# NethermindEth/latticefold

Hardware: AMD Instinct MI355X
Metric: folding-prover steps/sec (one NIFSProver::prove per step), GoldilocksRingNTT (higher is better)
Workload: dtype u64; 1 GPU; C4: GoldilocksRingNTT R1CS->CCS, m=N=2^20 rows, wit_len=262144, L=4, B=2^16, b=2, K=16, kappa=26, t=3; parallelism=replicas x1

## Files before the change

### latticefold_amd/api.py

```python
import ctypes as C
import os

import numpy as np

RE = 24
P = 2**64 - 2**32 + 1
RING_IDS = {"goldilocks": 0, "babybear": 1}
RING_WORDS = {"goldilocks": 24, "babybear": 72}
RING_TAU = {"goldilocks": 3, "babybear": 9}
FORMS = {"ntt": 0, "coeff": 1}
_HERE = os.path.dirname(os.path.abspath(__file__))
_SO = os.path.join(_HERE, "liblfhip.so")

u64p = C.POINTER(C.c_uint64)
u32p = C.POINTER(C.c_uint32)


EXCHANGE_FN = C.CFUNCTYPE(C.c_int, C.c_void_p, u64p, u64p, C.c_size_t)


class LfError(RuntimeError):
    def __init__(self, code, where=""):
        self.code = code
        msg = _lib().lf_strerror(code).decode() if _LIB is not None else str(code)
# ... 515 lines not shown
    def phase_ms(self):
        out = (C.c_float * 8)()
        _chk(_lib().lf_last_phase_ms(self.h, out), "lf_last_phase_ms")
        return {_lib().lf_phase_name(i).decode(): float(out[i]) for i in range(8)}

    def fold_paths(self):
        m = C.c_uint()
        _chk(_lib().lf_last_fold_paths(self.h, C.byref(m)), "lf_last_fold_paths")
        return m.value

    def lin_split_rounds(self):
        m = C.c_uint()
        _chk(_lib().lf_last_lin_split_rounds(self.h, C.byref(m)), "lf_last_lin_split_rounds")
        return m.value

    def fold_split_rounds(self):
        m = C.c_uint()
        _chk(_lib().lf_last_fold_split_rounds(self.h, C.byref(m)), "lf_last_fold_split_rounds")
        return m.value

    def timeline(self):
        names, ms = C.create_string_buffer(32 * 64), (C.c_double * 64)()
        n = _lib().lf_last_timeline(self.h, names, ms, 64)
        if n < 0:
            raise LfError(n, "lf_last_timeline")
        return [(names.raw[32 * i:32 * i + 32].split(b"\0")[0].decode(), float(ms[i])) for i in range(n)]

    def device_memory(self):
        f, t = C.c_size_t(), C.c_size_t()
        _chk(_lib().lf_device_memory(self.h, C.byref(f), C.byref(t)), "lf_device_memory")
# ... 574 lines not shown
```

### latticefold_amd/csrc/lf_capi.cpp

```cpp
#include "lf_ring_host.h"
#include <thread>
#include <vector>

const char *lf_strerror(int code) {
    switch (code) {
        case LF_OK: return "ok";
        case LF_ERR_INVALID: return "invalid argument / wrong length";
        case LF_ERR_HIP: return "HIP runtime error (no GPU or out of device memory)";
        case LF_ERR_UNSUPPORTED: return "unsupported parameter";
        case LF_ERR_BAD_TABLES: return "ring tables are not a ring isomorphism";
        case LF_ERR_NORM: return "witness coefficient exceeds the decomposition bound";
        case LF_ERR_SIZE_BOUNDS: return "invalid size bounds (m must be >= wit_len*L, power of two)";
        case LF_ERR_STATE: return "call sequence misuse";
        case LF_ERR_REJECT: return "verifier rejected the proof";
    }
    return "unknown error";
}
const char *lf_phase_name(int i) { return (i >= 0 && i < LF_N_PHASES) ? PHASE_NAMES[i] : ""; }

static int install_tables(lf_ctx *c, u64 nonres, const u64 *y) {
    CrtTables T;
    if (build_crt_tables(nonres, y, T) != 0) return LF_ERR_BAD_TABLES;
    c->ring.T = T;
    c->dcrt = make_dev_crt(T);
// ... 1009 lines not shown
        if (n >= max_marks) break;
        const char *w = m.first;
        while (*w == ' ') w++;
        snprintf(names + 32 * n, 32, "%s", w);
        ms[n++] = m.second;
    }
    return n;
}
int lf_abi_version(void) { return LFHIP_ABI_VERSION; }
int lf_debug_i8_prof(uint64_t *out64) {
    if (!out64) return LF_ERR_INVALID;
    return getenv("LF_I8G_PROF") ? ajtai_i8g_read_prof((unsigned long long *)out64) : ajtai_i8_read_prof((unsigned long long *)out64);
}
extern "C" int lfdbg_i8g_wg(unsigned int *out512) { return out512 ? ajtai_i8g_read_wg(out512) : -1; }
extern "C" unsigned lfdbg_i8g_planes_base(int ring, uint64_t base) { return ajtai_i8g_planes_base(ring == LF_RING_BABYBEAR ? ajtai_i8_babybear() : ajtai_i8_goldilocks(), base); }
int lf_last_fold_paths(lf_ctx *c, unsigned *sv_round_mask) {
    if (!c || !sv_round_mask) return LF_ERR_INVALID;
    *sv_round_mask = c->core_any().sv_round_mask;
    return LF_OK;
}
int lf_last_fold_split_rounds(lf_ctx *c, unsigned *round_mask) {
    if (!c || !round_mask) return LF_ERR_INVALID;
    *round_mask = c->core_any().fold_split_mask;
    return LF_OK;
}
int lf_last_lin_split_rounds(lf_ctx *c, unsigned *rounds) {
    if (!c || !rounds) return LF_ERR_INVALID;
    *rounds = c->bb ? 0u : c->lin_split_rounds;
    return LF_OK;
}
// ... 45 lines not shown
```

### latticefold_amd/csrc/lf_common.h

```cpp
#pragma once
#include <hip/hip_runtime.h>

#include <stdlib.h>

#include <atomic>

#include "../../include/lfhip.h"

#define HIPCHK(x)                                    \
    do {                                             \
        hipError_t e__ = (x);                        \
        if (e__ != hipSuccess) return LF_ERR_HIP;    \
    } while (0)
#define RET(x)                      \
    do {                            \
        int rc__ = (x);             \
        if (rc__ != LF_OK) return rc__; \
    } while (0)

extern "C" void lfplus_scratch_trim(int device);
template <class T> static inline hipError_t lf_dev_malloc(T **p, size_t bytes) {
    hipError_t e = hipMalloc((void **)p, bytes);
    if (e != hipErrorOutOfMemory) return e;
    (void)hipGetLastError();
// ... 43 lines not shown
    uint64_t *w_ccs = nullptr;
    size_t w_bytes = 0;
};

int lf_planes_alloc(lf_ctx *ctx, size_t bytes, int32_t **out);
void lf_planes_release(lf_ctx *ctx, size_t bytes, int32_t *p);
int lf_ctx_device(const lf_ctx *ctx);


struct Tunables {
    bool lin_u_eval = false, fold_unfused = false, fold_no_lut = false, fold_tab_r1 = false, theta_eval = false, fold_no_r4tab = false, fold_no_r5tab = false;
    bool fold_rounds_no_split = false;
    bool fold_sv_no_split = false;
    bool lin_no_split = false;
    size_t lin_split_min = (size_t)1 << 17;
    size_t fold_split_min = 8192;
    bool force_exchange = false;
    bool device_transcript = false;
    bool shard_plain_rounds = false;
    int shard_two_lanes = -1;
    size_t shard_lin_min = 16384;
    size_t shard_fold_min = 2048;
    long i8_wgs = 0;
    bool lin_no_r1cs = false;
    bool lin_no_small = false;
    size_t dot_min = 4096;
    bool dot_valu = false;
    bool fold_no_sv = false;
    size_t sv_min = 65536;
    int sv_rounds = 3;
// ... 1 lines not shown
    size_t fuse_min = 16384, lut_min = (size_t)1 << 17, tab_min = 16384;
    size_t r5_min = 8192;
    size_t tail_n = 2048;
    static Tunables read(size_t lut_min_default) {
        Tunables t;
        t.lut_min = lut_min_default;
        const char *e;
        t.lin_u_eval = getenv("LF_LIN_U_EVAL") != nullptr;
        t.fold_unfused = getenv("LF_FOLD_UNFUSED") != nullptr;
        t.fold_no_lut = getenv("LF_FOLD_NO_LUT") != nullptr;
        t.fold_tab_r1 = getenv("LF_FOLD_TAB_R1") != nullptr;
        t.fold_no_r4tab = getenv("LF_FOLD_NO_R4TAB") != nullptr;
        t.fold_no_r5tab = getenv("LF_FOLD_NO_R5TAB") != nullptr;
        t.lin_no_split = getenv("LF_LIN_NO_SPLIT") != nullptr;
        t.fold_sv_no_split = getenv("LF_FOLD_SV_NO_SPLIT") != nullptr;
        t.fold_rounds_no_split = getenv("LF_FOLD_ROUNDS_NO_SPLIT") != nullptr;
        if (const char *e = getenv("LF_LIN_SPLIT_MIN")) t.lin_split_min = (size_t)atoll(e);
        if (const char *e = getenv("LF_FOLD_SPLIT_MIN")) t.fold_split_min = (size_t)atoll(e);
        t.theta_eval = getenv("LF_THETA_EVAL") != nullptr;
        t.no_tail = getenv("LF_NO_TAIL") != nullptr;
        t.fold_no_sv = getenv("LF_FOLD_NO_SV") != nullptr;
        t.dot_valu = getenv("LF_DOT_VALU") != nullptr;
        if ((e = getenv("LF_DOT_MIN"))) t.dot_min = (size_t)atoll(e);
        t.lin_no_small = getenv("LF_LIN_NO_SMALL") != nullptr;
        t.lin_no_r1cs = getenv("LF_LIN_NO_R1CS") != nullptr;
        if ((e = getenv("LF_FOLD_SV_MIN"))) t.sv_min = (size_t)atoll(e);
        if ((e = getenv("LF_FOLD_SV_ROUNDS"))) t.sv_rounds = atoi(e);
        if ((e = getenv("LF_I8_WGS"))) t.i8_wgs = atol(e);
        if ((e = getenv("LF_SHARD_TWO_LANES"))) t.shard_two_lanes = atoi(e) != 0;
        if ((e = getenv("LF_SHARD_LIN_MIN"))) t.shard_lin_min = (size_t)atoll(e);
// ... 79 lines not shown
```

### latticefold_amd/csrc/lf_ctx.h

```cpp
#pragma once
#include <hip/hip_runtime.h>
#include <assert.h>
#include <string.h>

#include <atomic>
#include <chrono>
#include <condition_variable>
#include <functional>
#include <future>
#include <thread>
#include <map>
#include <memory>
#include <mutex>
#include <set>
#include <string>
#include <vector>

#include "../../include/lfhip.h"
#include "bb_capi.h"
#include "lf_ctx_core.h"
#include "lf_common.h"
#include "lf_dist.h"
#include "lf_kernels.h"
#include "lf_sb.h"
#include "lf_verify.h"

using namespace lf;

namespace lf {
void launch_fix_many(const DevCrt &t, const u64 *in, size_t ld_in, u64 *out, size_t ld_out, size_t n_in, u32 rows3, Fq3Const r, hipStream_t s);
}

#include <stdio.h>
#include <stdlib.h>
static bool lf_trace_on() { static int v = -1; if (v < 0) v = getenv("LF_TRACE") ? 1 : 0; return v == 1; }
#define LF_TRACE(c, msg)                                                              \
    do {                                                                              \
        if (lf_trace_on()) {                                                          \
// ... 103 lines not shown
    std::atomic<int> io_jobs{0};
    inline CtxCoreBase &core_any();
    bool have_ccs_any() { return core_any().have_ccs; }
    const lf_params &params_any() { return core_any().P; }
    size_t n_any() { return core_any().n; }
    size_t m_any() { return core_any().m; }
    size_t N_any() { return core_any().N; }
    HostRing ring;
    DevCrt dcrt;
    LaneWorker lane1;
    int agreed_two_lanes = -1;
    bool two_lanes_ok = false;
    lfdist::Comm comm[2];
    lfdist::Comm &cm() { assert(t_lane < 2); return comm[t_lane]; }
    bool ccs_general = false;
    size_t shc_r0 = (size_t)-1, shc_rcnt = 0, shc_lo = 0, shc_hi = 0;
    LinCombDesc desc{};
    std::vector<std::pair<const char *, double>> tl_marks;
    const lf_witness *bits_wit[2] = {nullptr, nullptr};
    u32 *bits_ptr[2] = {nullptr, nullptr};
    hipEvent_t bits_ev[2] = {nullptr, nullptr};
    hipEvent_t ev_yR = nullptr, ev_yL = nullptr;
    u64 *h_pin2 = nullptr;
    size_t h_pin2_words = 0;
    int pin2(size_t words) {
        if (words <= h_pin2_words) return LF_OK;
        if (h_pin2) (void)hipHostFree(h_pin2);
        h_pin2 = nullptr; h_pin2_words = 0;
        if (hipHostMalloc((void **)&h_pin2, words * 8) != hipSuccess) return LF_ERR_HIP;
        h_pin2_words = words;
        return LF_OK;
    }
    hipStream_t st_aux = nullptr;
    hipEvent_t ev_aux = nullptr;
    u64 *h_aux = nullptr;
    unsigned lin_split_rounds = 0;

    unsigned char *stage[LF_NLANES] = {nullptr, nullptr, nullptr};
    size_t stage_off[LF_NLANES] = {0, 0, 0};
    static constexpr size_t STAGE_BYTES = (size_t)1 << 20;
    int h2d_small(void *dst, const void *src, size_t bytes) {
        unsigned char *&ring = stage[t_lane];
        if (!ring && hipHostMalloc((void **)&ring, STAGE_BYTES, hipHostMallocDefault) != hipSuccess) { ring = nullptr; return LF_ERR_HIP; }
        const size_t need = (bytes + 63) & ~(size_t)63;
        if (need > STAGE_BYTES) {
            HIPCHK(hipMemcpyAsync(dst, src, bytes, hipMemcpyHostToDevice, stream()));
            HIPCHK(hipStreamSynchronize(stream()));
            return LF_OK;
        }
        if (stage_off[t_lane] + need > STAGE_BYTES) {
            HIPCHK(hipStreamSynchronize(stream()));
// ... 164 lines not shown
```

### latticefold_amd/csrc/lf_fold.cpp

```cpp
#include "lf_ring_host.h"

static int tail_host_rounds(lf_ctx *c, Transcript &tr, u32 epoch, u32 nr, u32 npts, bool dev_transcript, u64 *msgs, Fq3 *pt,
                            const std::function<void(u32)> *after_round = nullptr, u32 round0 = 0) {
    TailMail *mail = c->tail_mail;
    const auto t_start = std::chrono::steady_clock::now();
    double host_us = 0, wait_us = 0;
    auto t_mark = t_start;
    const bool tl_on = t_tl && t_tl->on;
    for (u32 i = 0; i < nr; i++) {
        u32 spins = 0;
        while (__atomic_load_n(&mail->msg_seq[i], __ATOMIC_ACQUIRE) != epoch) {
            __builtin_ia32_pause();
            if ((++spins & 0xfff) == 0) {
                if (__atomic_load_n(&mail->err, __ATOMIC_RELAXED) == epoch ||
                    std::chrono::duration<double>(std::chrono::steady_clock::now() - t_start).count() > 10.0) {
                    __atomic_store_n(&mail->abort_seq, epoch, __ATOMIC_RELEASE);
                    (void)hipStreamSynchronize(c->stream());
                    return LF_ERR_HIP;
                }
            }
        }
        if (tl_on) { auto nw = std::chrono::steady_clock::now(); wait_us += std::chrono::duration<double, std::micro>(nw - t_mark).count(); t_mark = nw; }
        u64 *evs = msgs + (size_t)i * npts * 24;
        memcpy(evs, (const void *)mail->msg[i], (size_t)npts * 24 * 8);
// ... 240 lines not shown
    od = od_host = c->round_out();
    if (!od) return LF_ERR_HIP;
    if (c->sh_world > 1) {
        RET(c->tbuf("fold_round_out", 5 * 24 + 8, &od_shard));
        od = od_shard;
    }
    const bool shard_tabs = shard_keep(c, 1, m);
    const size_t g_r0 = shard_tabs ? (size_t)c->sh_rank * (m / (size_t)c->sh_world) : 0, g_rcnt = shard_tabs ? m / (size_t)c->sh_world : (size_t)-1;
    size_t zc_lo = 0, zc_hi = n;
    if (shard_tabs) RET(shard_col_range(c, g_r0, g_rcnt, &zc_lo, &zc_hi));
    {
        hipStream_t s0 = c->stream(), s1 = (t_lane == 0) ? c->st_lane[1] : s0;
        u64 *zz1 = zz;
        if (s1 != s0) RET(c->tbuf("fold_zz1", (size_t)P.t * 24 * n, &zz1));
        RET(c->fork(s0, s1));
        for (int sd = 0; sd < 2; sd++) {
            hipStream_t st = sd ? s1 : s0;
            RET(side_mz(sd, st, sd ? zz1 : zz, sd ? "spmv_zaos_R" : "spmv_zaos_L", zc_lo, zc_hi, g_r0, g_rcnt));
            launch_add_fhat_comb(c->dcrt, S[sd].planes, N, K, d_ap + (size_t)sd * K * 3, G[sd], m, st, g_r0, g_rcnt);
        }
        RET(c->join(s1, s0));
    }
    { HostTimer ht(c); lfs::draw_mu_beta<GoldV>(tr, K2, P.s, mu, beta); }
    TL_MARK(" fold challenges");
    RET(powers_mu());
    RET(build_eq_dev(c, beta.data(), P.s, eqb));
    sv_split = !c->tn.fold_sv_no_split && P.s >= 4 && m >= 256;
    if (sv_split) {
        RET(c->tbuf("fold_svE1", 3 * (m / 2), &svE[0]));
        RET(c->tbuf("fold_svE2", 3 * (m / 4), &svE[1]));
        RET(c->tbuf("fold_svE3", 3 * (m / 8), &svE[2]));
        RET(build_eq_dev(c, beta.data() + 1, P.s - 1, svE[0]));
// ... 429 lines not shown
```

### latticefold_amd/csrc/lf_kernels.h

```cpp
#pragma once
#include "lf_ajtai_i8.h"
#include "lf_sv_rounds.h"
#include <hip/hip_runtime.h>

#include "lf_host.h"

namespace lf {

struct DevCrt {
    u64 nu;
    int nu2p40;
    u64 w4, w2, w10, w1, w7, w5, w11;
    int slot_of_pos[8], pos1[8], pos2[8];
    u64 tw1[8], tw2[8];
};
DevCrt make_dev_crt(const CrtTables &T);

struct Fq3Const { u64 c[3]; };

struct XbMat3 { u64 m[9]; };
void launch_aos_to_soa(const u64 *aos, u64 *soa, size_t n, hipStream_t s, u32 *flag = nullptr, const XbMat3 *Ti = nullptr);
void launch_soa_to_aos(const u64 *soa, u64 *aos, size_t n, hipStream_t s, const u32 *unless_flag = nullptr, const XbMat3 *T = nullptr);
void launch_ext_to_aos(const u64 *soa, u64 *aos, size_t n, hipStream_t s, const XbMat3 *T = nullptr);
void launch_slot_const_check(const u64 *tab, size_t n, u32 *flag, hipStream_t s);
// ... 33 lines not shown
                      u64 *zaos, u64 *out, size_t m, int accumulate, hipStream_t s, size_t r0 = 0, size_t rcnt = (size_t)-1);
void launch_spmv_t_eq(const DevCrt &t, const u32 *colptr, const u32 *rowidx, const u64 *val, const u64 *eq, size_t m,
                      u64 *q, size_t n, hipStream_t s, size_t c0 = 0, size_t ccnt = (size_t)-1 );
void launch_dot_batch(const DevCrt &t, const u64 *X, size_t ldx, u32 na, const u64 *Y, size_t ldy, u32 nb, size_t n,
                      u64 *partial, u64 *out, hipStream_t s);
size_t dot_partial_words(u32 na, u32 nb);
void launch_dot_eq(const DevCrt &t, const u64 *X, size_t ldx, u32 na, const u64 *eq, size_t ldeq, size_t n, u64 *partial,
                   u64 *out, hipStream_t s);
void launch_coef_eval(const DevCrt &t, const int32_t *planes, size_t n, const u64 *eq, size_t ldeq, u32 K, int mode_bits,
                      u64 *partial, u64 *out, hipStream_t s, size_t ldp = 0);
size_t coef_eval_partial_words(u32 K);
void launch_lincomb_z(const DevCrt &t, const u64 *z, size_t ldz, u32 K, const Fq3Const *coef_dev , u32 tt, size_t n,
                      u64 *out, hipStream_t s, u32 per_slot = 0);
void launch_add_fhat_comb(const DevCrt &t, const int32_t *planes, size_t n_planes, u32 K, const Fq3Const *apow_dev ,
                          u64 *G, size_t m, hipStream_t s, size_t r0 = 0, size_t rcnt = (size_t)-1 );

void launch_fix_ring(const DevCrt &t, const u64 *in, u64 *out, size_t n_in, Fq3Const r, hipStream_t s);
void launch_fix_fq3(const DevCrt &t, const u64 *in, u64 *out, size_t n_in, Fq3Const r, hipStream_t s);
size_t dot_i8_yb_bytes(size_t n);
size_t dot_i8_part_words(size_t n);
size_t dot_i8_tot_words();
int launch_dot_batch_i8(const DevCrt &t, const u64 *X, size_t ldx, u32 na, const u64 *Y, size_t ldy, u32 nb, size_t n, unsigned char *YB, int32_t *part,
                        long long *tot, u64 *out, hipStream_t s, bool y_packed = false, u32 nb_out = 0, u32 b0 = 0);
int launch_dot_pack_y(const u64 *X, const u64 *Y, size_t ldy, u32 nb, size_t n, unsigned char *YB, hipStream_t s);
void launch_vs_combine(const u64 *vs , u32 K, u64 *v , hipStream_t s);
void launch_fix_final(const DevCrt &t, const u64 *in , u32 rows3, Fq3Const r, u64 *out , hipStream_t s);

struct LinCombDesc {
    u32 t, q;
    u32 S_off[9];
// ... 114 lines not shown
```

### latticefold_amd/csrc/lf_kernels.hip

```cpp
#include "lf_kernels.h"

#include <stdlib.h>

#include "lf_kernels_dev.cuh"
#include "lf_sb.h"

namespace lf {


DevCrt make_dev_crt(const CrtTables &T) {
    DevCrt d;
    d.nu = T.nu; d.nu2p40 = T.nu_is_2p40;
    d.w4 = T.w4; d.w2 = T.w2; d.w10 = T.w10; d.w1 = T.w1; d.w7 = T.w7; d.w5 = T.w5; d.w11 = T.w11;
    for (int p = 0; p < 8; p++) {
        d.slot_of_pos[p] = T.slot_of_pos[p]; d.pos1[p] = T.pos1[p]; d.pos2[p] = T.pos2[p];
        d.tw1[p] = T.tw1[p]; d.tw2[p] = T.tw2[p];
    }
    return d;
}


__global__ void __launch_bounds__(256) k_modsum(const u64 *parts, u32 nparts, size_t words, u64 *out) {
    size_t w = (size_t)blockIdx.x * 256 + threadIdx.x;
    if (w >= words) return;
// ... 680 lines not shown
            const u64 *e = T[(d * NQ + q) * 16 + ((mg >> (4 * q)) & 15)];
            part = fq3_add(part, fq3_make(e[0], e[1], e[2]));
        }
        acc = v < 0 ? fq3_sub(acc, part) : fq3_add(acc, part);
    }
    st3(G, m, slot, row, acc);
}
void launch_add_fhat_comb(const DevCrt &t, const int32_t *planes, size_t n_planes, u32 K, const Fq3Const *apow_dev, u64 *G, size_t m,
                          hipStream_t s, size_t r0, size_t rcnt) {
    size_t r1 = rcnt == (size_t)-1 ? n_planes : (r0 + rcnt < n_planes ? r0 + rcnt : n_planes);
    if (rcnt == (size_t)-1) r0 = 0;
    if (r1 <= r0) return;
    if (K <= 16) hipLaunchKernelGGL(k_add_fhat_comb<4>, dim3(cdiv(r1 - r0, 256), 8), dim3(256), 0, s, planes, n_planes, K, apow_dev, G, m, r0, r1);
    else hipLaunchKernelGGL(k_add_fhat_comb<8>, dim3(cdiv(r1 - r0, 256), 8), dim3(256), 0, s, planes, n_planes, K, apow_dev, G, m, r0, r1);
}

template <bool NU>
__global__ void __launch_bounds__(256) k_fix(DevCrt t, const u64 *in, size_t ld_in, u64 *out, size_t ld_out, size_t n_out, Fq3Const r) {
    size_t j = (size_t)blockIdx.x * 256 + threadIdx.x;
    size_t row = blockIdx.y;
    if (j >= n_out) return;
    const u64 *p = in + row * 3 * ld_in;
    Fq3 rr = fq3_make(r.c[0], r.c[1], r.c[2]);
    ulonglong2 a0 = *(const ulonglong2 *)(p + 2 * j), a1 = *(const ulonglong2 *)(p + ld_in + 2 * j), a2 = *(const ulonglong2 *)(p + 2 * ld_in + 2 * j);
    Fq3 v0 = fq3_make(a0.x, a1.x, a2.x), v1 = fq3_make(a0.y, a1.y, a2.y);
    Fq3 res = fq3_add(v0, M3<NU>(fq3_sub(v1, v0), rr, t.nu));
    u64 *q = out + row * 3 * ld_out;
    q[j] = res.c[0]; q[ld_out + j] = res.c[1]; q[2 * ld_out + j] = res.c[2];
}
void launch_fix_ring(const DevCrt &t, const u64 *in, u64 *out, size_t n_in, Fq3Const r, hipStream_t s) {
// ... 67 lines not shown
```

### latticefold_amd/csrc/lf_prove.cpp

```cpp
#include "lf_ring_host.h"


static int run_lin_sumcheck(lf_ctx *c, Transcript &tr, const u64 *mz, const u64 *eqb, u64 *msgs , Fq3 *point, u64 *u_dev = nullptr,
                            const std::function<void(u32)> *after_round = nullptr, const Fq3 *beta = nullptr) {
    const lf_params &P = c->P;
    u32 deg = P.d + 1;
    size_t m = c->m;
    u64 *fx[2], *fe[2], *partial, *od;
    RET(c->tbuf("lin_fix0", (size_t)P.t * 24 * (m / 2), &fx[0]));
    RET(c->tbuf("lin_fix1", (size_t)P.t * 24 * (m / 4 ? m / 4 : 1), &fx[1]));
    RET(c->tbuf("lin_efix0", 3 * (m / 2), &fe[0]));
    RET(c->tbuf("lin_efix1", 3 * (m / 4 ? m / 4 : 1), &fe[1]));
    RET(c->tbuf("round_partial", round_partial_words(), &partial));
    od = c->round_out();
    if (!od) return LF_ERR_HIP;
    { HostTimer ht(c); lfs::sumcheck_prologue<GoldV>(tr, P.s, deg); }
    const u64 *cur = mz, *cure = eqb;
    size_t n = m;
    int flip = 0;
    const size_t Gw = (size_t)c->sh_world, gr = (size_t)c->sh_rank;
    bool sharded = shard_keep(c, 0, m);
    u64 *od_dev = nullptr;
    if (Gw > 1) RET(c->tbuf("lin_round_out", (size_t)(deg + 1) * 24 + 8, &od_dev));
    const u32 dT = P.d;
    const bool wide = P.t > 4 || P.d > 3;
    bool split = beta && Gw == 1 && !c->tn.lin_no_split && P.s >= 2 && m >= c->tn.lin_split_min && m >= 16 && dT >= 1 && deg <= 8;
    const GoldV hv{c->ring};
    lfs::SplitCoef<GoldV> sp = lfs::split_coef(hv, fq3_one(), beta ? beta[0] : fq3_one());
    if (split) RET(build_eq_dev(c, beta + 1, P.s - 1, fe[0]));
    c->lin_split_rounds = 0;
    for (u32 round = 1; round <= P.s; round++) {
        if (split && round >= 2) {
            const bool tail_next = !wide && !c->tn.no_tail && n <= c->tn.tail_n && n >= 4 && P.s - round + 1 <= TAIL_MAX_ROUNDS;
            const lfs::SplitCoef<GoldV> sp_next = lfs::split_coef(hv, c->ring.mul3(sp.c, lfs::eq1(hv, beta[round - 2], point[round - 2])), beta[round - 1]);
            if (tail_next || n < 8 || n / 2 < c->tn.lin_split_min || !sp_next.ok) {
                u64 *ex;
                RET(c->tbuf("lin_eexp", 3 * n, &ex));
                const Fq3 bi = beta[round - 2];
                launch_eq_expand(c->dcrt, cure, n / 2, n / 2, f3c(c->ring.mul3(sp.c, fq3_sub(fq3_one(), bi))), f3c(c->ring.mul3(sp.c, bi)), ex, n, c->stream());
                cure = ex;
                split = false;
            } else sp = sp_next;
        }
        if (!wide && !sharded && !c->tn.no_tail && round >= 2 && n <= c->tn.tail_n && n >= 4 && P.s - round + 1 <= TAIL_MAX_ROUNDS) {
            int trc = lin_tail_rounds(c, tr, cur, cure, n, fx[flip], partial, round, point, msgs, deg, after_round);
            if (trc == LF_OK) { cur = fx[flip]; n = 2; break; }
            if (trc != LF_ERR_UNSUPPORTED) return trc;
        }
        bool fused_now = false;
        const u64 *prev = cur, *preve = cure;
        size_t prevn = n;
        if (round > 1) {
            Fq3Const r = f3c(point[round - 2]);
            if (sharded) {
                const size_t e0 = gr * (n / Gw), ecnt = n / Gw;
                launch_fix_many(c->dcrt, cur + e0, n, fx[flip] + e0 / 2, n / 2, ecnt, P.t * 8, r, c->stream());
                launch_fix_many(c->dcrt, cure + e0, n, fe[flip] + e0 / 2, n / 2, ecnt, 1, r, c->stream());
            } else if (split || (Gw == 1 && n >= 8)) {
                fused_now = true;
            } else {
                launch_fix_many(c->dcrt, cur, n, fx[flip], n / 2, n, P.t * 8, r, c->stream());
                launch_fix_many(c->dcrt, cure, n, fe[flip], n / 2, n, 1, r, c->stream());
            }
            cur = fx[flip]; cure = split ? fe[(round - 1) & 1] : fe[flip];
            flip ^= 1;
            n /= 2;
            if (sharded && !shard_keep(c, 0, n)) {
                const size_t lcl = n / Gw;
                const GatherPart gp[2] = {{cur + gr * lcl, n, (u64 *)cur, (size_t)P.t * 24}, {cure + gr * lcl, n, (u64 *)cure, 3}};
                RET(gather_parts(c, gp, 2, lcl));
                sharded = false;
            }
        }
        u64 *ev = msgs + (size_t)(round - 1) * (deg + 1) * 24;
        if (sharded) {
            const size_t p0 = gr * (n / 2 / Gw), pcnt = n / 2 / Gw;
            launch_lin_round(c->dcrt, c->desc, cur + 2 * p0, n, cure + 2 * p0, n, 2 * pcnt, deg, partial, od_dev, c->stream(), c->lin_blocks);
            RET(exchange_modsum_dev(c, od_dev, (size_t)(deg + 1) * 24));
            HIPCHK(hipMemcpyAsync(od, od_dev, (size_t)(deg + 1) * 24 * 8, hipMemcpyDeviceToHost, c->stream()));
        } else if (split) {
            const u32 xmask = round == 1 ? (1u << (dT + 1)) - 1 : (((1u << (dT + 1)) - 1) & ~2u);
            if (round == 1) launch_lin_round(c->dcrt, c->desc, cur, n, fe[0], n / 2, n, deg, partial, od, c->stream(), c->lin_blocks, xmask);
            else launch_lin_round_fused(c->dcrt, c->desc, prev, prevn, preve, prevn / 2, f3c(point[round - 2]), (u64 *)cur, n, (u64 *)cure, n / 2, n, deg, partial, od, c->stream(),
                                        c->lin_blocks, xmask);
            if (round == 1) cure = fe[0];
        } else if (fused_now)
            launch_lin_round_fused(c->dcrt, c->desc, prev, prevn, preve, prevn, f3c(point[round - 2]), (u64 *)cur, n, (u64 *)cure, n, n, deg, partial, od, c->stream(), c->lin_blocks);
        else launch_lin_round(c->dcrt, c->desc, cur, n, cure, n, n, deg, partial, od, c->stream(), c->lin_blocks);
        RET(c->lane_sync());
        if (split) {
            HostTimer ht2(c);
            c->lin_split_rounds++;
            lfs::complete_lin_split(hv, sp, dT, od, round >= 2 ? msgs + (size_t)(round - 2) * (deg + 1) * 24 : nullptr, point[round >= 2 ? round - 2 : 0], ev);
        } else
        memcpy(ev, od, (size_t)(deg + 1) * 24 * 8);
        HostTimer ht(c);
        point[round - 1] = lfs::sumcheck_round<GoldV>(tr, ev, deg + 1);
        if (after_round) (*after_round)(round);
        if (round <= 2 || round == 4 || round == 8) TL_MARK_ROUND("  lin round", round);
    }
    TL_MARK("  lin rounds done");
    if (u_dev) launch_fix_final(c->dcrt, cur, P.t * 8, f3c(point[P.s - 1]), u_dev, c->stream());
    return LF_OK;
// ... 51 lines not shown
    RET(c->tbuf("lin_z", 24 * n, &z));
    RET(c->tbuf("lin_mz", (size_t)P.t * 24 * m, &mz));
    RET(c->tbuf("lin_eqb", 3 * m, &eqb));
    RET(c->tbuf("eq_r_R", 3 * m, &eqr));
    RET(c->tbuf("red_partial", 256 * 4096, &partial));
    RET(c->tbuf("lin_small", 4096, &od));
    RET(build_z(c, wit->planes, 1, 0, head.data(), z));
    TL_MARK("  lin z enqueued");
    std::vector<Fq3> beta(P.s);
    {
        HostTimer ht(c);
        tr.absorb_label("beta_s");
        for (u32 i = 0; i < P.s; i++) beta[i] = tr.get_challenge();
    }
    RET(build_eq_dev(c, beta.data(), P.s, eqb));
    {
        const size_t Gw = (size_t)c->sh_world;
        const bool rows_sliced = shard_keep(c, 0, m) && !c->tn.lin_u_eval;
        const size_t r0 = rows_sliced ? (size_t)c->sh_rank * (m / Gw) : 0, rcnt = rows_sliced ? m / Gw : m;
        if (c->ccs_general) {
            u64 *zaos;
            RET(c->tbuf("spmv_zaos", (size_t)P.t * n * 24, &zaos));
            launch_soa_to_aos(z, zaos, n, c->stream());
            for (u32 j = 0; j < P.t; j++)
                launch_spmv_rows(c->dcrt, 1, &c->d_rowptr[j], &c->d_col[j], &c->d_val[j], nullptr, 0, n, zaos, mz + (size_t)j * 24 * m, m, 0, c->stream(), r0, rcnt);
        } else
        for (u32 j = 0; j < P.t; j++)
            launch_spmv(c->dcrt, c->d_rowptr[j], c->d_col[j], c->d_val[j], z, n, mz + (size_t)j * 24 * m, m, 0, c->stream(), r0, rcnt);
    }
    std::vector<Fq3> pt(P.s);
    const bool u_eval = c->tn.lin_u_eval;
    TL_MARK("  lin Mz enqueued");
    struct VsSplit {
        bool armed = false, launched = false, failed = false;
// ... 24 lines not shown
    }
    const std::function<void(u32)> vs_hook = [&](u32 round) {
        if (!vsp.armed || round != vsp.J) return;
        Fq3Const *h = (Fq3Const *)c->h_aux;
        for (u32 i = 0; i < vsp.J; i++) h[i] = f3c(pt[i]);
        bool ok = hipMemcpyAsync(vsp.rd, h, vsp.J * sizeof(Fq3Const), hipMemcpyHostToDevice, c->st_aux) == hipSuccess;
        if (ok) {
            launch_build_eq2(c->dcrt, vsp.rd, vsp.J, vsp.scr, vsp.eqlo, c->st_aux);
            ok = hipStreamWaitEvent(c->st_aux, c->bits_ev[vsp.sd], 0) == hipSuccess &&
                 launch_sv_vs_blocks(c->bits_ptr[vsp.sd], c->N, vsp.eqlo, (size_t)1 << vsp.J, vsp.J, P.K, vsp.EB, vsp.part, c->st_aux) == 0 &&
                 hipEventRecord(c->ev_aux, c->st_aux) == hipSuccess;
        }
        vsp.launched = ok;
        vsp.failed = !ok;
    };
    RET(run_lin_sumcheck(c, tr, mz, eqb, proof, pt.data(), u_eval ? nullptr : od + 72, vsp.armed ? &vs_hook : nullptr, beta.data()));
    if (vsp.failed) { (void)hipStreamSynchronize(c->st_aux); return LF_ERR_HIP; }
    if (!vsp.launched) RET(build_eq_dev(c, pt.data(), P.s, eqr));
    u64 *v = proof + (size_t)P.s * (P.d + 2) * 24, *u = v + 3 * 24;
    {
        size_t i0, cnt;
        shard_slice(c, c->N, &i0, &cnt);
        c->vs_wit = nullptr;
        if (P.b == 2 && c->sh_world == 1 && !c->tn.force_exchange) {
            u64 *vs;
            RET(c->tbuf("lin_vs", (size_t)P.K * 72 + 8, &vs));
            if (vsp.launched) {
                std::vector<u64> w((size_t)3 * vsp.nblocks);
                for (u32 b = 0; b < vsp.nblocks; b++) {
                    Fq3 acc = fq3_one();
                    for (u32 j = 0; vsp.J + j < P.s; j++) acc = c->ring.mul3(acc, ((b >> j) & 1) ? pt[vsp.J + j] : fq3_sub(fq3_one(), pt[vsp.J + j]));
// ... 524 lines not shown
```

### latticefold_amd/csrc/lf_ring_host.h

```cpp
#pragma once
#include "bb_ctx.h"
#include "lf_check.h"
#include "lf_ctx.h"
#include "lf_dev_ptr.h"
#include "lf_mlsumcheck.h"
#include "lf_witness_parts.h"

#pragma GCC visibility push(hidden)
inline size_t lcccs_len(const lf_params *p, size_t tau) { return (size_t)p->s + tau + p->kappa + p->t + p->l + 1; }
inline size_t cccs_len(const lf_params *p) { return (size_t)p->kappa + p->l; }
inline size_t lin_proof_len(const lf_params *p, size_t tau) { return (size_t)p->s * (p->d + 2) + tau + p->t; }
inline size_t dec_proof_len(const lf_params *p, size_t tau) { return (size_t)p->K * (p->t + tau + p->l + 1 + p->kappa); }
inline size_t fold_proof_len(const lf_params *p, size_t tau) { return (size_t)p->s * (2 * p->b + 1) + 2 * (size_t)p->K * (tau + p->t); }
inline size_t proof_len(const lf_params *p, size_t tau) { return lin_proof_len(p, tau) + 2 * dec_proof_len(p, tau) + fold_proof_len(p, tau); }

namespace lfring {
using namespace lf;
using namespace lfbb;

template <class Ctx> struct Ring;
template <> struct Ring<lf_ctx> {
    typedef u64 W;
    typedef u64 Part;
    typedef Fq3 Ext;
// ... 427 lines not shown
            void *dcp = dalloc(c->d_colptr, (n + 1) * 4), *dri = dalloc(c->d_rowidx, (nnz + 1) * 4), *dvT = dalloc(c->d_valT, (nnz + 1) * RE * sizeof(W));
            if (!drp || !dci || !dv || !dcp || !dri || !dvT) return LF_ERR_HIP;
            HIPCHK(hipMemcpy(drp, rowptr[j], (m + 1) * 4, hipMemcpyHostToDevice));
            HIPCHK(hipMemcpy(dci, col[j], nnz * 4, hipMemcpyHostToDevice));
            HIPCHK(hipMemcpy(dv, v, nnz * RE * sizeof(W), hipMemcpyHostToDevice));
            HIPCHK(hipMemcpy(dcp, cp.data(), (n + 1) * 4, hipMemcpyHostToDevice));
            HIPCHK(hipMemcpy(dri, ri.data(), nnz * 4, hipMemcpyHostToDevice));
            HIPCHK(hipMemcpy(dvT, vT.data(), nnz * RE * sizeof(W), hipMemcpyHostToDevice));
        }
        if constexpr (R::general_csr) {
            const size_t rows_used = n < m ? n : m;
            c->ccs_general = false;
            for (u32 jj = 0; jj < P->t; jj++)
                if ((size_t)rowptr[jj][m] * 2 > rows_used * 3) c->ccs_general = true;
            c->shc_r0 = (size_t)-1;
        }
        c->have_ccs = true;
        return LF_OK;
    }

    static int ajtai_commit(C *c, const u64 *f, size_t n, size_t batch, u64 *out, Origin org = Origin::host) {
        std::lock_guard<std::mutex> g(c->mu);
        if (!c->A_loaded) return LF_ERR_STATE;
        if (n != c->nA_total) return LF_ERR_INVALID;
        HIPCHK(hipSetDevice(c->device));
        DevIo<C> io(c, org);
        RET(io.array(f, batch * n));
        W *F;
        u64 *o;
        RET(c->tbuf("io_a", batch * n * RE, &F));
// ... 755 lines not shown
```

Measured before the change: 59.97 steps/s.

## Skip trailing empty CCS rows in linearization sumcheck and fuse fold g-row build

Computes the number of live (non-empty) CCS rows when loading the constraint system and pads it to a granule. The linearization sumcheck then processes only the live prefix in its early rounds, zero-filling the dead tail once halving stops lining up. The fold step also gains a single fused kernel that does the sparse matrix-vector product and the f-hat combination per row, replacing the separate SpMV and add passes. This adds bookkeeping for the live/padded row count and new kernel variants, and relies on the dead rows being exactly zero in every affected buffer.

Result: faster. 62.52 steps/s, median of 6 (+4.3%).

```diff
diff --git a/latticefold_amd/api.py b/latticefold_amd/api.py
--- a/latticefold_amd/api.py
+++ b/latticefold_amd/api.py
@@ -553,6 +553,16 @@
         _chk(_lib().lf_last_lin_split_rounds(self.h, C.byref(m)), "lf_last_lin_split_rounds")
         return m.value
 
+    def live_rows(self):
+        f = _lib().lfdbg_live_rows
+        f.argtypes, f.restype = [C.c_void_p], C.c_longlong
+        return f(self.h)
+
+    def lin_live_rounds(self):
+        f = _lib().lfdbg_last_lin_live_rounds
+        f.argtypes, f.restype = [C.c_void_p], C.c_int
+        return f(self.h)
+
     def fold_split_rounds(self):
         m = C.c_uint()
         _chk(_lib().lf_last_fold_split_rounds(self.h, C.byref(m)), "lf_last_fold_split_rounds")
diff --git a/latticefold_amd/csrc/lf_capi.cpp b/latticefold_amd/csrc/lf_capi.cpp
--- a/latticefold_amd/csrc/lf_capi.cpp
+++ b/latticefold_amd/csrc/lf_capi.cpp
@@ -1047,6 +1047,13 @@
 }
 extern "C" int lfdbg_i8g_wg(unsigned int *out512) { return out512 ? ajtai_i8g_read_wg(out512) : -1; }
 extern "C" unsigned lfdbg_i8g_planes_base(int ring, uint64_t base) { return ajtai_i8g_planes_base(ring == LF_RING_BABYBEAR ? ajtai_i8_babybear() : ajtai_i8_goldilocks(), base); }
+extern "C" long long lfdbg_live_rows(lf_ctx *c) { return c && !c->bb && c->have_ccs ? (long long)c->live_rows : -1; }
+extern "C" size_t lfdbg_live_rows_csr(unsigned t, size_t m, const uint32_t *const *rowptr) { return lflive::live_rows(t, m, rowptr); }
+extern "C" void lfdbg_live_schedule(size_t m, size_t live, int low, unsigned rounds, size_t *out) {
+    const lflive::Plan p = low ? lflive::plan(m, live, lflive::GRANULE_LOW, lflive::MIN_M_LOW) : lflive::plan(m, live, lflive::GRANULE, lflive::MIN_M);
+    for (unsigned i = 1; i <= rounds; i++) out[i - 1] = lflive::entries(p, i);
+}
+extern "C" int lfdbg_last_lin_live_rounds(lf_ctx *c) { return c && !c->bb ? (int)c->lin_live_rounds : -1; }
 int lf_last_fold_paths(lf_ctx *c, unsigned *sv_round_mask) {
     if (!c || !sv_round_mask) return LF_ERR_INVALID;
     *sv_round_mask = c->core_any().sv_round_mask;
diff --git a/latticefold_amd/csrc/lf_common.h b/latticefold_amd/csrc/lf_common.h
--- a/latticefold_amd/csrc/lf_common.h
+++ b/latticefold_amd/csrc/lf_common.h
@@ -81,6 +81,8 @@
     bool fold_sv_no_split = false;
     bool lin_no_split = false;
     size_t lin_split_min = (size_t)1 << 17;
+    bool no_live_rows = false;
+    bool live_rows_low = false;
     size_t fold_split_min = 8192;
     bool force_exchange = false;
     bool device_transcript = false;
@@ -112,6 +114,8 @@
         t.fold_no_r5tab = getenv("LF_FOLD_NO_R5TAB") != nullptr;
         t.lin_no_split = getenv("LF_LIN_NO_SPLIT") != nullptr;
         t.fold_sv_no_split = getenv("LF_FOLD_SV_NO_SPLIT") != nullptr;
+        t.no_live_rows = getenv("LF_NO_LIVE_ROWS") != nullptr;
+        t.live_rows_low = getenv("LF_LIVE_ROWS_LOW") != nullptr;
         t.fold_rounds_no_split = getenv("LF_FOLD_ROUNDS_NO_SPLIT") != nullptr;
         if (const char *e = getenv("LF_LIN_SPLIT_MIN")) t.lin_split_min = (size_t)atoll(e);
         if (const char *e = getenv("LF_FOLD_SPLIT_MIN")) t.fold_split_min = (size_t)atoll(e);
diff --git a/latticefold_amd/csrc/lf_ctx.h b/latticefold_amd/csrc/lf_ctx.h
--- a/latticefold_amd/csrc/lf_ctx.h
+++ b/latticefold_amd/csrc/lf_ctx.h
@@ -22,6 +22,7 @@
 #include "lf_common.h"
 #include "lf_dist.h"
 #include "lf_kernels.h"
+#include "lf_live_rows.h"
 #include "lf_sb.h"
 #include "lf_verify.h"
 
@@ -155,6 +156,11 @@
     lfdist::Comm comm[2];
     lfdist::Comm &cm() { assert(t_lane < 2); return comm[t_lane]; }
     bool ccs_general = false;
+    size_t live_rows = 0;
+    lflive::Plan live_plan() const {
+        if (tn.no_live_rows || sh_world > 1) return lflive::plan(m, m, 0, 0);
+        return tn.live_rows_low ? lflive::plan(m, live_rows, lflive::GRANULE_LOW, lflive::MIN_M_LOW) : lflive::plan(m, live_rows, lflive::GRANULE, lflive::MIN_M);
+    }
     size_t shc_r0 = (size_t)-1, shc_rcnt = 0, shc_lo = 0, shc_hi = 0;
     LinCombDesc desc{};
     std::vector<std::pair<const char *, double>> tl_marks;
@@ -176,6 +182,7 @@
     hipEvent_t ev_aux = nullptr;
     u64 *h_aux = nullptr;
     unsigned lin_split_rounds = 0;
+    unsigned lin_live_rounds = 0;
 
     unsigned char *stage[LF_NLANES] = {nullptr, nullptr, nullptr};
     size_t stage_off[LF_NLANES] = {0, 0, 0};
diff --git a/latticefold_amd/csrc/lf_fold.cpp b/latticefold_amd/csrc/lf_fold.cpp
--- a/latticefold_amd/csrc/lf_fold.cpp
+++ b/latticefold_amd/csrc/lf_fold.cpp
@@ -278,8 +278,16 @@
         u64 *zz1 = zz;
         if (s1 != s0) RET(c->tbuf("fold_zz1", (size_t)P.t * 24 * n, &zz1));
         RET(c->fork(s0, s1));
+        const bool one_pass = !c->tn.no_live_rows && !c->ccs_general && P.t <= 4 && !shard_tabs && c->sh_world == 1 && N <= m;
         for (int sd = 0; sd < 2; sd++) {
             hipStream_t st = sd ? s1 : s0;
+            if (one_pass) {
+                u64 *zb = sd ? zz1 : zz;
+                launch_lincomb_z(c->dcrt, S[sd].z, n, K, d_zp + (size_t)sd * K * P.t, P.t, n, zb, st);
+                launch_g_rows(c->dcrt, P.t, c->d_rowptr.data(), c->d_col.data(), c->d_val.data(), zb, (size_t)24 * n, n, c->live_rows, S[sd].planes, N, K,
+                              d_ap + (size_t)sd * K * 3, G[sd], m, st);
+                continue;
+            }
             RET(side_mz(sd, st, sd ? zz1 : zz, sd ? "spmv_zaos_R" : "spmv_zaos_L", zc_lo, zc_hi, g_r0, g_rcnt));
             launch_add_fhat_comb(c->dcrt, S[sd].planes, N, K, d_ap + (size_t)sd * K * 3, G[sd], m, st, g_r0, g_rcnt);
         }
diff --git a/latticefold_amd/csrc/lf_kernels.h b/latticefold_amd/csrc/lf_kernels.h
--- a/latticefold_amd/csrc/lf_kernels.h
+++ b/latticefold_amd/csrc/lf_kernels.h
@@ -71,6 +71,8 @@
                       u64 *out, hipStream_t s, u32 per_slot = 0);
 void launch_add_fhat_comb(const DevCrt &t, const int32_t *planes, size_t n_planes, u32 K, const Fq3Const *apow_dev ,
                           u64 *G, size_t m, hipStream_t s, size_t r0 = 0, size_t rcnt = (size_t)-1 );
+void launch_g_rows(const DevCrt &t, u32 nm, const u32 *const *rowptr, const u32 *const *col, const u64 *const *val, const u64 *z, size_t z_stride, size_t ldz, size_t live,
+                   const int32_t *planes, size_t n_planes, u32 K, const Fq3Const *apow_dev , u64 *G, size_t m, hipStream_t s);
 
 void launch_fix_ring(const DevCrt &t, const u64 *in, u64 *out, size_t n_in, Fq3Const r, hipStream_t s);
 void launch_fix_fq3(const DevCrt &t, const u64 *in, u64 *out, size_t n_in, Fq3Const r, hipStream_t s);
diff --git a/latticefold_amd/csrc/lf_kernels.hip b/latticefold_amd/csrc/lf_kernels.hip
--- a/latticefold_amd/csrc/lf_kernels.hip
+++ b/latticefold_amd/csrc/lf_kernels.hip
@@ -718,6 +718,66 @@
     if (K <= 16) hipLaunchKernelGGL(k_add_fhat_comb<4>, dim3(cdiv(r1 - r0, 256), 8), dim3(256), 0, s, planes, n_planes, K, apow_dev, G, m, r0, r1);
     else hipLaunchKernelGGL(k_add_fhat_comb<8>, dim3(cdiv(r1 - r0, 256), 8), dim3(256), 0, s, planes, n_planes, K, apow_dev, G, m, r0, r1);
 }
+template <bool NU, int NQ>
+__global__ void __launch_bounds__(256) k_g_rows(DevCrt t, SpmvSet ms, size_t ldz, size_t live, const int32_t *planes, size_t n_planes, u32 K, const Fq3Const *apow, u64 *G,
+                                                size_t m) {
+    __shared__ u64 T[3 * NQ * 16][4];
+    for (u32 e = threadIdx.x; e < 3 * NQ * 16; e += 256) {
+        u32 val = e % 16, q = (e / 16) % NQ, d = e / (16 * NQ);
+        Fq3 sum = fq3_zero();
+        for (u32 b = 0; b < 4; b++)
+            if (4 * q + b < K && ((val >> b) & 1)) {
+                Fq3Const a = apow[(4 * q + b) * 3 + d];
+                sum = fq3_add(sum, fq3_make(a.c[0], a.c[1], a.c[2]));
+            }
+        T[e][0] = sum.c[0]; T[e][1] = sum.c[1]; T[e][2] = sum.c[2]; T[e][3] = 0;
+    }
+    __syncthreads();
+    const size_t row = (size_t)blockIdx.x * 256 + threadIdx.x;
+    const u32 slot = blockIdx.y;
+    if (row >= m) return;
+    Fq3 acc = fq3_zero();
+    if (row < live) {
+#pragma unroll
+        for (u32 j = 0; j < 4; j++) {
+            if (j < ms.nm) {
+                const u32 *rp = ms.rowptr[j], *cl = ms.col[j];
+                for (u32 k = rp[row]; k < rp[row + 1]; k++) {
+                    const u64 *v = ms.val[j] + (size_t)k * 24 + 3 * slot;
+                    acc = fq3_add(acc, M3<NU>(fq3_make(v[0], v[1], v[2]), ld3(ms.z[j], ldz, slot, cl[k]), t.nu));
+                }
+            }
+        }
+    }
+    if (row < n_planes) {
+#pragma unroll
+        for (int d = 0; d < 3; d++) {
+            int32_t v = planes[(size_t)(8 * d + slot) * n_planes + row];
+            u32 mg = (u32)(v < 0 ? -v : v);
+            Fq3 part = fq3_zero();
+#pragma unroll
+            for (int q = 0; q < NQ; q++) {
+                const u64 *e = T[(d * NQ + q) * 16 + ((mg >> (4 * q)) & 15)];
+                part = fq3_add(part, fq3_make(e[0], e[1], e[2]));
+            }
+            acc = v < 0 ? fq3_sub(acc, part) : fq3_add(acc, part);
+        }
+    }
+    st3(G, m, slot, row, acc);
+}
+void launch_g_rows(const DevCrt &t, u32 nm, const u32 *const *rowptr, const u32 *const *col, const u64 *const *val, const u64 *z, size_t z_stride, size_t ldz, size_t live,
+                   const int32_t *planes, size_t n_planes, u32 K, const Fq3Const *apow_dev, u64 *G, size_t m, hipStream_t s) {
+    if (!m || nm > 4 || n_planes > m) return;
+    SpmvSet ms = {};
+    ms.nm = nm;
+    for (u32 j = 0; j < nm; j++) { ms.rowptr[j] = rowptr[j]; ms.col[j] = col[j]; ms.val[j] = val[j]; ms.z[j] = z + (size_t)j * z_stride; }
+    if (live > m) live = m;
+    const dim3 grid(cdiv(m, 256), 8);
+#define LF_GR(NUV, NQ) hipLaunchKernelGGL((k_g_rows<NUV, NQ>), grid, dim3(256), 0, s, t, ms, ldz, live, planes, n_planes, K, apow_dev, G, m)
+    if (K <= 16) { if (t.nu2p40) LF_GR(true, 4); else LF_GR(false, 4); }
+    else { if (t.nu2p40) LF_GR(true, 8); else LF_GR(false, 8); }
+#undef LF_GR
+}
 
 template <bool NU>
 __global__ void __launch_bounds__(256) k_fix(DevCrt t, const u64 *in, size_t ld_in, u64 *out, size_t ld_out, size_t n_out, Fq3Const r) {
diff --git a/latticefold_amd/csrc/lf_live_rows.h b/latticefold_amd/csrc/lf_live_rows.h
--- /dev/null
+++ b/latticefold_amd/csrc/lf_live_rows.h
@@ -0,0 +1,45 @@
+#pragma once
+#include <stddef.h>
+#include <stdint.h>
+
+namespace lflive {
+
+static constexpr size_t GRANULE = 4096;
+static constexpr size_t MIN_M = (size_t)1 << 14;
+static constexpr size_t GRANULE_LOW = 8, MIN_M_LOW = 16;
+
+static inline size_t live_rows(unsigned t, size_t m, const uint32_t *const *rowptr) {
+    size_t live = 0;
+    for (unsigned j = 0; j < t; j++) {
+        size_t r = m;
+        while (r > live && rowptr[j][r] == rowptr[j][r - 1]) r--;
+        if (r > live) live = r;
+    }
+    return live;
+}
+
+struct Plan {
+    size_t m = 0;
+    size_t pad = 0;
+    bool on() const { return pad < m; }
+};
+static inline Plan plan(size_t m, size_t live, size_t granule, size_t min_m) {
+    Plan p;
+    p.m = m; p.pad = m;
+    if (granule < 4 || (granule & (granule - 1)) || m < min_m || live > m) return p;
+    size_t pad = (live + granule - 1) / granule * granule;
+    if (pad < granule) pad = granule;
+    if (pad <= m / 2) p.pad = pad;
+    return p;
+}
+static inline bool halves(size_t n, size_t nl) { return nl < n && nl % 4 == 0 && nl >= 4; }
+static inline size_t entries(const Plan &p, unsigned round) {
+    size_t n = p.m, nl = p.pad;
+    for (unsigned i = 1; i < round; i++) {
+        nl = halves(n, nl) ? nl / 2 : n / 2;
+        n /= 2;
+    }
+    return nl;
+}
+
+}
diff --git a/latticefold_amd/csrc/lf_prove.cpp b/latticefold_amd/csrc/lf_prove.cpp
--- a/latticefold_amd/csrc/lf_prove.cpp
+++ b/latticefold_amd/csrc/lf_prove.cpp
@@ -2,7 +2,7 @@
 
 
 static int run_lin_sumcheck(lf_ctx *c, Transcript &tr, const u64 *mz, const u64 *eqb, u64 *msgs , Fq3 *point, u64 *u_dev = nullptr,
-                            const std::function<void(u32)> *after_round = nullptr, const Fq3 *beta = nullptr) {
+                            const std::function<void(u32)> *after_round = nullptr, const Fq3 *beta = nullptr, size_t live = 0) {
     const lf_params &P = c->P;
     u32 deg = P.d + 1;
     size_t m = c->m;
@@ -18,6 +18,7 @@
     const u64 *cur = mz, *cure = eqb;
     size_t n = m;
     int flip = 0;
+    size_t nl = live && live < m && c->sh_world == 1 ? live : m;
     const size_t Gw = (size_t)c->sh_world, gr = (size_t)c->sh_rank;
     bool sharded = shard_keep(c, 0, m);
     u64 *od_dev = nullptr;
@@ -29,6 +30,7 @@
     lfs::SplitCoef<GoldV> sp = lfs::split_coef(hv, fq3_one(), beta ? beta[0] : fq3_one());
     if (split) RET(build_eq_dev(c, beta + 1, P.s - 1, fe[0]));
     c->lin_split_rounds = 0;
+    c->lin_live_rounds = 0;
     for (u32 round = 1; round <= P.s; round++) {
         if (split && round >= 2) {
             const bool tail_next = !wide && !c->tn.no_tail && n <= c->tn.tail_n && n >= 4 && P.s - round + 1 <= TAIL_MAX_ROUNDS;
@@ -42,7 +44,12 @@
                 split = false;
             } else sp = sp_next;
         }
-        if (!wide && !sharded && !c->tn.no_tail && round >= 2 && n <= c->tn.tail_n && n >= 4 && P.s - round + 1 <= TAIL_MAX_ROUNDS) {
+        const bool tail_now = !wide && !sharded && !c->tn.no_tail && round >= 2 && n <= c->tn.tail_n && n >= 4 && P.s - round + 1 <= TAIL_MAX_ROUNDS;
+        if (round >= 2 && nl < n && !(lflive::halves(n, nl) && !tail_now && !sharded && (split || (Gw == 1 && n >= 8)))) {
+            HIPCHK(hipMemset2DAsync((u64 *)cur + nl, n * 8, 0, (n - nl) * 8, (size_t)P.t * 24, c->stream()));
+            nl = n;
+        }
+        if (tail_now) {
             int trc = lin_tail_rounds(c, tr, cur, cure, n, fx[flip], partial, round, point, msgs, deg, after_round);
             if (trc == LF_OK) { cur = fx[flip]; n = 2; break; }
             if (trc != LF_ERR_UNSUPPORTED) return trc;
@@ -65,6 +72,7 @@
             cur = fx[flip]; cure = split ? fe[(round - 1) & 1] : fe[flip];
             flip ^= 1;
             n /= 2;
+            nl /= 2;
             if (sharded && !shard_keep(c, 0, n)) {
                 const size_t lcl = n / Gw;
                 const GatherPart gp[2] = {{cur + gr * lcl, n, (u64 *)cur, (size_t)P.t * 24}, {cure + gr * lcl, n, (u64 *)cure, 3}};
@@ -73,6 +81,7 @@
             }
         }
         u64 *ev = msgs + (size_t)(round - 1) * (deg + 1) * 24;
+        if (nl < n) c->lin_live_rounds++;
         if (sharded) {
             const size_t p0 = gr * (n / 2 / Gw), pcnt = n / 2 / Gw;
             launch_lin_round(c->dcrt, c->desc, cur + 2 * p0, n, cure + 2 * p0, n, 2 * pcnt, deg, partial, od_dev, c->stream(), c->lin_blocks);
@@ -80,13 +89,16 @@
             HIPCHK(hipMemcpyAsync(od, od_dev, (size_t)(deg + 1) * 24 * 8, hipMemcpyDeviceToHost, c->stream()));
         } else if (split) {
             const u32 xmask = round == 1 ? (1u << (dT + 1)) - 1 : (((1u << (dT + 1)) - 1) & ~2u);
-            if (round == 1) launch_lin_round(c->dcrt, c->desc, cur, n, fe[0], n / 2, n, deg, partial, od, c->stream(), c->lin_blocks, xmask);
-            else launch_lin_round_fused(c->dcrt, c->desc, prev, prevn, preve, prevn / 2, f3c(point[round - 2]), (u64 *)cur, n, (u64 *)cure, n / 2, n, deg, partial, od, c->stream(),
+            if (round == 1) launch_lin_round(c->dcrt, c->desc, cur, n, fe[0], n / 2, nl, deg, partial, od, c->stream(), c->lin_blocks, xmask);
+            else launch_lin_round_fused(c->dcrt, c->desc, prev, prevn, preve, prevn / 2, f3c(point[round - 2]), (u64 *)cur, n, (u64 *)cure, n / 2, nl, deg, partial, od, c->stream(),
                                         c->lin_blocks, xmask);
             if (round == 1) cure = fe[0];
-        } else if (fused_now)
-            launch_lin_round_fused(c->dcrt, c->desc, prev, prevn, preve, prevn, f3c(point[round - 2]), (u64 *)cur, n, (u64 *)cure, n, n, deg, partial, od, c->stream(), c->lin_blocks);
-        else launch_lin_round(c->dcrt, c->desc, cur, n, cure, n, n, deg, partial, od, c->stream(), c->lin_blocks);
+            else if (nl < n) launch_eq_pairsum(preve + nl, prevn / 2, (n - nl) / 2, (u64 *)cure + nl / 2, n / 2, c->stream());
+        } else if (fused_now) {
+            launch_lin_round_fused(c->dcrt, c->desc, prev, prevn, preve, prevn, f3c(point[round - 2]), (u64 *)cur, n, (u64 *)cure, n, nl, deg, partial, od, c->stream(), c->lin_blocks);
+            if (nl < n) launch_fix_many(c->dcrt, preve + 2 * nl, prevn, (u64 *)cure + nl, n, prevn - 2 * nl, 1, f3c(point[round - 2]), c->stream());
+        }
+        else launch_lin_round(c->dcrt, c->desc, cur, n, cure, n, nl, deg, partial, od, c->stream(), c->lin_blocks);
         RET(c->lane_sync());
         if (split) {
             HostTimer ht2(c);
@@ -168,10 +180,11 @@
         for (u32 i = 0; i < P.s; i++) beta[i] = tr.get_challenge();
     }
     RET(build_eq_dev(c, beta.data(), P.s, eqb));
+    const size_t live = c->tn.lin_u_eval ? m : c->live_plan().pad;
     {
         const size_t Gw = (size_t)c->sh_world;
         const bool rows_sliced = shard_keep(c, 0, m) && !c->tn.lin_u_eval;
-        const size_t r0 = rows_sliced ? (size_t)c->sh_rank * (m / Gw) : 0, rcnt = rows_sliced ? m / Gw : m;
+        const size_t r0 = rows_sliced ? (size_t)c->sh_rank * (m / Gw) : 0, rcnt = rows_sliced ? m / Gw : live;
         if (c->ccs_general) {
             u64 *zaos;
             RET(c->tbuf("spmv_zaos", (size_t)P.t * n * 24, &zaos));
@@ -226,7 +239,7 @@
         vsp.launched = ok;
         vsp.failed = !ok;
     };
-    RET(run_lin_sumcheck(c, tr, mz, eqb, proof, pt.data(), u_eval ? nullptr : od + 72, vsp.armed ? &vs_hook : nullptr, beta.data()));
+    RET(run_lin_sumcheck(c, tr, mz, eqb, proof, pt.data(), u_eval ? nullptr : od + 72, vsp.armed ? &vs_hook : nullptr, beta.data(), live));
     if (vsp.failed) { (void)hipStreamSynchronize(c->st_aux); return LF_ERR_HIP; }
     if (!vsp.launched) RET(build_eq_dev(c, pt.data(), P.s, eqr));
     u64 *v = proof + (size_t)P.s * (P.d + 2) * 24, *u = v + 3 * 24;
diff --git a/latticefold_amd/csrc/lf_ring_host.h b/latticefold_amd/csrc/lf_ring_host.h
--- a/latticefold_amd/csrc/lf_ring_host.h
+++ b/latticefold_amd/csrc/lf_ring_host.h
@@ -465,6 +465,7 @@
             for (u32 jj = 0; jj < P->t; jj++)
                 if ((size_t)rowptr[jj][m] * 2 > rows_used * 3) c->ccs_general = true;
             c->shc_r0 = (size_t)-1;
+            c->live_rows = lflive::live_rows(P->t, m, rowptr);
         }
         c->have_ccs = true;
         return LF_OK;
```
